# LemonATsu/UNet-PhaseGen

Hardware: AMD Instinct MI355X
Metric: spectrogram-frames/sec (train fwd+bwd) (higher is better)
Workload: dtype f32; 1 GPU; train.py full step (fwd + cos/sin/mag loss + bwd + Adam), UNetModel(1024, 2048), per-GPU batch 64 x 1024 bins x 256 frames (BASELINE configs[2]); global_batch=64, frames=256, channels=1024, parallelism=dp1, grad_allreduce_payload=fp32, adam=fused into the wgrad epilogues

## Files before the change

### unet-phasegen_amd/csrc/conv_raw_wgrad.hip

```cpp
#include "conv_common.h"

namespace {

template <int KW, int S> struct GRaw {
    static constexpr int WL = 15 * S + KW;
    static constexpr int WLP = g_wlp(KW, S);
    static constexpr int NQT = RBN / KW;
    static constexpr int TNV = NQT * KW;
    static constexpr int SUB = NQT * WLP;
    static constexpr int SUBS = (SUB + 63) / 64 * 64;
    static constexpr int NE = (SUB + NT - 1) / NT;
    static constexpr int STG = RTILE_A + 2 * SUBS;
    static constexpr int SUBP = (SUB + 255) / 256 * 256;
    static_assert(WL <= WLP, "window does not fit its slot");
};

template <int KW, int S, int BF>
__device__ __forceinline__ void g_raw_bf(const IgemmParams& p) {
    using C = GRaw<KW, S>;
    __shared__ __attribute__((aligned(16))) float lds[2 * C::STG];
    const int tid = threadIdx.x, lane = tid & 63;
    const int wv = __builtin_amdgcn_readfirstlane(tid >> 6), wm = wv >> 1, wn = wv & 1;
    const int kt = dma_kt(lane, wv);
    const rsrc_t rp = make_rsrc(p.pt, p.pt_bytes), rx = make_rsrc(p.x, p.x_bytes);
// ... 50 lines not shown
            }
        }
        int bbase[4];
#pragma unroll
        for (int jb = 0; jb < 4; ++jb) {
            const int c = wn * 128 + jb * 32 + (lane & 31), qc = c / KW;
            bbase[jb] = qc * C::WLP + (c - qc * KW) + S * 8 * (lane >> 5);
        }
        AccR acc;
#pragma unroll
        for (int i = 0; i < 2; ++i)
#pragma unroll
            for (int j = 0; j < 4; ++j)
#pragma unroll
                for (int r = 0; r < 16; ++r) acc.c[i][j][r] = 0.f;

        int gb, gi;
        { const int k0 = sb * BK; gb = k0 / p.LP; gi = k0 - gb * p.LP; }
        int kc_cur = 16;

#define GRAW_ISSUE(STAGE_PTR, K0)                                                                         \
    {   float* const As = (STAGE_PTR) + wv * 64; float* const Bw = (STAGE_PTR) + RTILE_A + wv * 64;       \
        const int k0 = (K0);                                                                              \
        const int kc = p.LP - gi;                            \
        if (FASTP && kc >= 16 && gb < p.B) {                                                              \
            const int sa = gb * pbs4 + gi * 4;                                                            \
            _Pragma("unroll") for (int e = 0; e < 2; ++e) dma16s(rp, As + wv * 192 + e * 1024, pv[FASTP ? e : 0], sa); \
        } else {                                                                                          \
          int bb, ii; divmod24(k0 + kt, p.LP, p.inv_LP, bb, ii);                                          \
          const int po = bb < p.B ? bb * pbs4 + ii * 4 : OOB;                                             \
          _Pragma("unroll") for (int e = 0; e < 8; ++e) dma4(rp, As + e * 256, aoff[e] + po); }           \
        const int w0 = S * gi - p.p;                             \
        if (FASTW && kc >= 16 && gb < p.B && w0 >= 0 && w0 + C::WLP <= p.Lx) {    \
            const int sw_ = gb * xbs4 + w0 * 4;                                                           \
            _Pragma("unroll") for (int e = 0; e < NE16; ++e)                                              \
                if (4 * (e * NT + wv * 64) < C::SUB) dma16s(rx, (STAGE_PTR) + RTILE_A + 4 * (e * NT + wv * 64), woff[FASTW ? e : 0], sw_); \
        } else {                                                                                          \
        const int sb0 = gb < p.B ? gb * xbs4 : -NEVER, sb1 = (kc < 16 && gb + 1 < p.B) ? (gb + 1) * xbs4 : -NEVER; \
        _Pragma("unroll") for (int e = 0; e < C::NE; ++e) {                                               \
            if ((e + 1) * NT <= C::SUB || e * NT + wv * 64 < C::SUB) {                                    \
                const int ps = S * gi + GRAW_VV(e);                                                       \
                dma4(rx, Bw + e * NT, ((unsigned)ps < (unsigned)p.Lx && sb0 >= 0) ? sb0 + GRAW_CHOFF(e) + ps * 4 : FAR); \
            }                                                                                             \
        }                                                                                                 \
        if (kc < 16) {                                  \
            _Pragma("unroll") for (int e = 0; e < C::NE; ++e) {                                           \
                if ((e + 1) * NT <= C::SUB || e * NT + wv * 64 < C::SUB) {                                                          \
                    const int ps = GRAW_VV(e);                                                            \
                    dma4(rx, Bw + C::SUBS + e * NT, ((unsigned)ps < (unsigned)p.Lx && sb1 >= 0) ? sb1 + GRAW_CHOFF(e) + ps * 4 : FAR); \
                }                                                                                         \
            }                                                                                             \
        }                                                                                                 \
        }                                                                                                 \
        kc_next = kc < 16 ? kc : 16;                                                                      \
        gi += BK; if (gi >= p.LP) { gi -= p.LP; ++gb; }                                                   \
    }

        PG_STAMP_DECL
        int kc_next;
        GRAW_ISSUE(lds, sb * BK)
        kc_cur = kc_next;
        __syncthreads();
        for (int sl = sb; sl < se; ++sl) {
            const int cur = (sl - sb) & 1;
            PG_STAMP(0)
#if defined(PG_G_ABL) && PG_G_ABL == 1
            kc_next = 16;
#else
            GRAW_ISSUE(lds + (cur ^ 1) * C::STG, (sl + 1) * BK)
#endif
            __builtin_amdgcn_sched_barrier(0);
            PG_STAMP(1)
            {
                const float* As = lds + cur * C::STG;
                const float* Bw = As + RTILE_A;
                const int r = lane & 31, h = lane >> 5, sw = (r >> 2) & 3;
                const float* ap = As + (wm * 64 + r) * BK;
                f32x4 a[2][2];
                float b[4][8];
                if (kc_cur >= 16) {
#pragma unroll
                    for (int i = 0; i < 2; ++i) a[i][0] = *reinterpret_cast<const f32x4*>(ap + i * 32 * BK + (((2 * h) ^ sw) << 2));
#pragma unroll
                    for (int ip = 0; ip < 4; ++ip) {
                        if (ip == 2) {
#pragma unroll
                            for (int i = 0; i < 2; ++i) a[i][1] = *reinterpret_cast<const f32x4*>(ap + i * 32 * BK + (((2 * h + 1) ^ sw) << 2));
                        }
#pragma unroll
                        for (int jb = 0; jb < 4; ++jb) { b[jb][2 * ip] = Bw[bbase[jb] + S * 2 * ip]; b[jb][2 * ip + 1] = Bw[bbase[jb] + S * (2 * ip + 1)]; }
                    }
                } else {
#pragma unroll
                    for (int c = 0; c < 2; ++c)
#pragma unroll
                        for (int i = 0; i < 2; ++i) a[i][c] = *reinterpret_cast<const f32x4*>(ap + i * 32 * BK + (((2 * h + c) ^ sw) << 2));
                    typedef const volatile __attribute__((address_space(3))) float* lds_vptr;
                    const lds_vptr Bv = (lds_vptr)Bw;
                    const int shift = C::SUBS - S * kc_cur;
#pragma unroll
                    for (int i = 0; i < 8; ++i) {
                        const int d = (8 * h + i >= kc_cur) ? shift : 0;
#pragma unroll
                        for (int jb = 0; jb < 4; ++jb) b[jb][i] = Bv[bbase[jb] + S * i + d];
                    }
                }
                if (slopeA != 1.0f) {
#pragma unroll
                    for (int i = 0; i < 2; ++i)
#pragma unroll
                        for (int c = 0; c < 2; ++c)
#pragma unroll
                            for (int v = 0; v < 4; ++v) a[i][c][v] = act_apply(a[i][c][v], slopeA);
                }
                if (slopeB != 1.0f) {
#pragma unroll
                    for (int jb = 0; jb < 4; ++jb)
#pragma unroll
                        for (int i = 0; i < 8; ++i) b[jb][i] = act_apply(b[jb][i], slopeB);
                }
                if (BF) mfma_low_2x4<BF>(a, b, acc);
                else {
#pragma unroll
                    for (int kk = 0; kk < 8; ++kk) {
#pragma unroll
                        for (int i = 0; i < 2; ++i)
#pragma unroll
                            for (int j = 0; j < 4; ++j)
                                acc.c[i][j] = __builtin_amdgcn_mfma_f32_32x32x2f32(a[i][kk >> 2][kk & 3], b[j][kk], acc.c[i][j], 0, 0, 0);
                    }
                }
            }
            __builtin_amdgcn_sched_barrier(0);
            PG_STAMP(2)
            kc_cur = kc_next;
#if defined(PG_G_ABL) && PG_G_ABL == 2
            asm volatile("s_waitcnt lgkmcnt(0)\n\ts_barrier" ::: "memory");
#else
            __syncthreads();
#endif
            PG_STAMP(3)
        }
        PG_STAMP_FLUSH
#undef GRAW_ISSUE
#undef GRAW_CHOFF
#undef GRAW_VV
        if (sb == 0 && se == p.nslab) epilogue_g<S, 2, 4>(p, acc, m0, n0, lane, wm, wn, n0 + C::TNV);
        else store_partial(p.ws, g, slot, acc, tid);
        pos += se - sb;
        slot = 1;
    }
}

template <int KW, int S, int BF>
__device__ __forceinline__ void g_ps_bf(const IgemmParams& p) {
    using C = GRaw<KW, S>;
    constexpr int STG = RTILE_A + (C::SUB + 255) / 256 * 256;
    constexpr int NE16 = (C::SUB / 4 + NT - 1) / NT;
    static_assert(C::WLP % 4 == 0 && C::WLP <= 64, "16-byte window pieces; channel 0 inside the first 64 floats");
    __shared__ __attribute__((aligned(16))) float lds[2 * STG];
    const int tid = threadIdx.x, lane = tid & 63;
    const int wv = __builtin_amdgcn_readfirstlane(tid >> 6), wm = wv >> 1, wn = wv & 1;
    const rsrc_t rp = make_rsrc(p.pt, p.pt_bytes), rx = make_rsrc(p.x, p.x_bytes);
    const float slopeA = act_slope(p.act_p), slopeB = act_slope(p.act_x);
    const int pbs4 = (int)p.pt_bs * 4, xbs4 = (int)p.x_bs * 4;
    const int cps = (p.LP + 15) >> 4;
    const int g = logical_wg(blockIdx.x, gridDim.x, p.whole);
    const Split sp = make_split(p.tilesM * p.tilesN, p.nslab, gridDim.x, p.whole);
    int pos = split_lo(sp, g);
    const int pos_end = split_lo(sp, g + 1);
    int slot = 0;
    while (pos < pos_end) {
        const int tile = pos / p.nslab, sb = pos - tile * p.nslab;
        const int se = min(p.nslab, sb + (pos_end - pos));
        const int m0 = (tile / p.tilesN) * RBM, n0 = (tile % p.tilesN) * C::TNV;
        const int qbase = (tile % p.tilesN) * C::NQT;

        int pv[2], woff[NE16];
#pragma unroll
        for (int e = 0; e < 2; ++e) {
            const int m = m0 + dma16_row(lane, wv, e);
            pv[e] = m < p.M ? (m * p.LP + dma16_kc(lane)) * 4 : FAR;
        }
#pragma unroll
        for (int e = 0; e < NE16; ++e) {
            const int f = 4 * (tid + NT * e), ql = f / C::WLP, v0 = f - ql * C::WLP;
            const int off = ((qbase + ql) * p.Lx + v0 - p.p) * 4;
            woff[e] = (f < C::SUB && qbase + ql < p.Q && off >= 0) ? off : FAR;
        }
        const bool fix0 = qbase == 0 && wv == 0;
        int f0_off, f0_v;
        { const int ql = lane / C::WLP, v = lane - ql * C::WLP; f0_off = ql < p.Q ? ql * p.Lx * 4 : FAR; f0_v = v - p.p; }
        int bbase[4], pj[4];
#pragma unroll
        for (int jb = 0; jb < 4; ++jb) {
            const int c = wn * 128 + jb * 32 + (lane & 31), qc = c / KW;
            bbase[jb] = qc * C::WLP + (c - qc * KW) + S * 8 * (lane >> 5);
            pj[jb] = (c - qc * KW) + S * 8 * (lane >> 5) - p.p;
        }
        AccR acc;
#pragma unroll
        for (int i = 0; i < 2; ++i)
#pragma unroll
            for (int j = 0; j < 4; ++j)
#pragma unroll
                for (int r = 0; r < 16; ++r) acc.c[i][j][r] = 0.f;

        int gb = sb / cps, gc = sb - gb * cps;
#define GPS_ISSUE(STAGE_PTR)                                                                              \
    {   float* const As = (STAGE_PTR) + wv * 64;                                                          \
        if (gb < p.B) {                                                                                   \
            const int gi = gc << 4;                                                                       \
            const int sa = gb * pbs4 + gi * 4;                                                            \
            _Pragma("unroll") for (int e = 0; e < 2; ++e) dma16s(rp, As + wv * 192 + e * 1024, pv[e], sa); \
            const int sw_ = gb * xbs4 + S * gi * 4;                                                       \
            _Pragma("unroll") for (int e = 0; e < NE16; ++e)                                              \
                if (4 * (e * NT + wv * 64) < C::SUB) dma16s(rx, (STAGE_PTR) + RTILE_A + 4 * (e * NT + wv * 64), woff[e], sw_); \
            if (fix0) {                                                                                   \
                const int ps = S * gi + f0_v;                                                             \
                dma4(rx, (STAGE_PTR) + RTILE_A, (unsigned)ps < (unsigned)p.Lx ? gb * xbs4 + f0_off + ps * 4 : FAR); \
            }                                                                                             \
        }                                                                                                 \
        if (++gc == cps) { gc = 0; ++gb; }                                                                \
    }
        int mb = gb, mc = gc;
        GPS_ISSUE(lds)
        __syncthreads();
        for (int sl = sb; sl < se; ++sl) {
            const int cur = (sl - sb) & 1;
            GPS_ISSUE(lds + (cur ^ 1) * STG)
            __builtin_amdgcn_sched_barrier(0);
            {
                const float* As = lds + cur * STG;
                const float* Bw = As + RTILE_A;
                const int r = lane & 31, h = lane >> 5, sw = (r >> 2) & 3;
                const float* ap = As + (wm * 64 + r) * BK;
                const int gi = mc << 4, kc = p.LP - gi;
                const int w0 = S * gi;
                f32x4 a[2][2];
                float b[4][8];
#pragma unroll
                for (int i = 0; i < 2; ++i) a[i][0] = *reinterpret_cast<const f32x4*>(ap + i * 32 * BK + (((2 * h) ^ sw) << 2));
#pragma unroll
                for (int ip = 0; ip < 4; ++ip) {
                    if (ip == 2) {
#pragma unroll
                        for (int i = 0; i < 2; ++i) a[i][1] = *reinterpret_cast<const f32x4*>(ap + i * 32 * BK + (((2 * h + 1) ^ sw) << 2));
                    }
#pragma unroll
                    for (int jb = 0; jb < 4; ++jb) { b[jb][2 * ip] = Bw[bbase[jb] + S * 2 * ip]; b[jb][2 * ip + 1] = Bw[bbase[jb] + S * (2 * ip + 1)]; }
                }
                if (kc < 16) {
#pragma unroll
                    for (int i = 0; i < 2; ++i)
#pragma unroll
                        for (int c = 0; c < 2; ++c)
#pragma unroll
                            for (int v = 0; v < 4; ++v) a[i][c][v] = (8 * h + 4 * c + v < kc) ? a[i][c][v] : 0.f;
                }
                if (w0 < p.p || w0 - p.p + C::WLP > p.Lx) {
#pragma unroll
                    for (int jb = 0; jb < 4; ++jb)
#pragma unroll
                        for (int i = 0; i < 8; ++i) b[jb][i] = (unsigned)(w0 + pj[jb] + S * i) < (unsigned)p.Lx ? b[jb][i] : 0.f;
                }
                if (slopeA != 1.0f) {
#pragma unroll
                    for (int i = 0; i < 2; ++i)
#pragma unroll
                        for (int c = 0; c < 2; ++c)
#pragma unroll
                            for (int v = 0; v < 4; ++v) a[i][c][v] = act_apply(a[i][c][v], slopeA);
                }
                if (slopeB != 1.0f) {
#pragma unroll
                    for (int jb = 0; jb < 4; ++jb)
#pragma unroll
                        for (int i = 0; i < 8; ++i) b[jb][i] = act_apply(b[jb][i], slopeB);
                }
                if (BF) mfma_low_2x4<BF>(a, b, acc);
                else {
#pragma unroll
                    for (int kk = 0; kk < 8; ++kk)
#pragma unroll
                        for (int i = 0; i < 2; ++i)
#pragma unroll
                            for (int j = 0; j < 4; ++j)
                                acc.c[i][j] = __builtin_amdgcn_mfma_f32_32x32x2f32(a[i][kk >> 2][kk & 3], b[j][kk], acc.c[i][j], 0, 0, 0);
                }
            }
            __builtin_amdgcn_sched_barrier(0);
            if (++mc == cps) { mc = 0; ++mb; }
            __syncthreads();
        }
#undef GPS_ISSUE
        (void)mb;
        if (sb == 0 && se == p.nslab) epilogue_g<S, 2, 4>(p, acc, m0, n0, lane, wm, wn, n0 + C::TNV);
        else store_partial(p.ws, g, slot, acc, tid);
        pos += se - sb;
        slot = 1;
    }
}

template <int KW, int S>
__device__ __forceinline__ void g_raw_f32(const IgemmParams& p) {
    using C = GRaw<KW, S>;
    constexpr int NP = 2 * C::SUBP / 4;
    constexpr int NE2 = (NP + NT - 1) / NT;
    constexpr int STG = RTILE_A + 2 * C::SUBP;
    static_assert(C::WLP % 4 == 0 && 2 * STG * 4 <= 64 * 1024, "16-byte window pieces; LDS budget");
    __shared__ __attribute__((aligned(16))) float lds[2 * STG];
    const int tid = threadIdx.x, lane = tid & 63;
    const int wv = __builtin_amdgcn_readfirstlane(tid >> 6), wm = wv >> 1, wn = wv & 1;
    const rsrc_t rp = make_rsrc(p.pk, p.pk_bytes), rx = make_rsrc(p.qk, p.qk_bytes);
    const int qbs4 = p.qk_bs * 4, klast4 = (p.nslab - 1) * BK * 4;
    const int g = logical_wg(blockIdx.x, gridDim.x, p.whole);
    const Split sp = make_split(p.tilesM * p.tilesN, p.nslab, gridDim.x, p.whole);
    int pos = split_lo(sp, g);
    const int pos_end = split_lo(sp, g + 1);
    int slot = 0;
    while (pos < pos_end) {
        const int tile = pos / p.nslab, sb = pos - tile * p.nslab;
        const int se = min(p.nslab, sb + (pos_end - pos));
        const int m0 = (tile / p.tilesN) * RBM, n0 = (tile % p.tilesN) * C::TNV;
        const int qbase = (tile % p.tilesN) * C::NQT;
        int pv[2], woff[NE2];
#pragma unroll
        for (int e = 0; e < 2; ++e) {
            const int m = m0 + dma16_row(lane, wv, e);
            pv[e] = m < p.M ? (m * p.Kp + dma16_kc(lane)) * 4 : FAR;
        }
#pragma unroll
        for (int e = 0; e < NE2; ++e) {
            const int pc = tid + NT * e, sub = pc >= C::SUBP / 4 ? 1 : 0, f = 4 * pc - sub * C::SUBP, ql = f / C::WLP, v0 = f - ql * C::WLP;
            woff[e] = (f < C::SUB && qbase + ql < p.Q) ? ((qbase + ql) * p.Lq + v0) * 4 : FAR;
        }
        int bbase[4];
#pragma unroll
        for (int jb = 0; jb < 4; ++jb) {
            const int c = wn * 128 + jb * 32 + (lane & 31), qc = c / KW;
            bbase[jb] = qc * C::WLP + (c - qc * KW) + S * 8 * (lane >> 5);
        }
        AccR acc;
#pragma unroll
        for (int i = 0; i < 2; ++i)
#pragma unroll
            for (int j = 0; j < 4; ++j)
#pragma unroll
                for (int r = 0; r < 16; ++r) acc.c[i][j][r] = 0.f;

        int gb, gi;
        { const int k0 = sb * BK; gb = k0 / p.LP; gi = k0 - gb * p.LP; }
        int kc_cur, kc_next;
#define GRF_ISSUE(STAGE_PTR, K0)                                                                          \
    {   const int sa = min((K0) * 4, klast4);                                                             \
        _Pragma("unroll") for (int e = 0; e < 2; ++e) dma16s(rp, (STAGE_PTR) + wv * 256 + e * 1024, pv[e], sa); \
        const int kc = p.LP - gi;                                                                         \
        const int sw0 = min(gb, p.B - 1) * qbs4 + S * gi * 4;                                             \
        const int sw1 = (kc < 16 && gb + 1 < p.B) ? (gb + 1) * qbs4 : sw0;                                \
        _Pragma("unroll") for (int e = 0; e < NE2; ++e) {                                                 \
            const int pc0 = e * NT + wv * 64;                                 \
            if ((e + 1) * NT <= NP || pc0 < NP)                                                           \
                dma16s(rx, (STAGE_PTR) + RTILE_A + 4 * pc0, woff[e], pc0 >= C::SUBP / 4 ? sw1 : sw0);     \
        }                                                                                                 \
        kc_next = kc < 16 ? kc : 16;                                                                      \
        gi += BK; if (gi >= p.LP) { gi -= p.LP; ++gb; }                                                   \
    }
        PG_STAMP_DECL
        GRF_ISSUE(lds, sb * BK)
        kc_cur = kc_next;
        __syncthreads();
        for (int sl = sb; sl < se; ++sl) {
            const int cur = (sl - sb) & 1;
            PG_STAMP(0)
#if defined(PG_G_ABL) && PG_G_ABL == 1
            kc_next = 16;
#else
            GRF_ISSUE(lds + (cur ^ 1) * STG, (sl + 1) * BK)
#endif
            __builtin_amdgcn_sched_barrier(0);
            PG_STAMP(1)
            {
                const float* As = lds + cur * STG;
                const float* Bw = As + RTILE_A;
                const int r = lane & 31, h = lane >> 5, sw = (r >> 2) & 3;
                const float* ap = As + (wm * 64 + r) * BK;
                f32x4 a[2][2];
                float b[4][8];
                if (kc_cur >= 16) {
#pragma unroll
                    for (int i = 0; i < 2; ++i) a[i][0] = *reinterpret_cast<const f32x4*>(ap + i * 32 * BK + (((2 * h) ^ sw) << 2));
#pragma unroll
                    for (int ip = 0; ip < 4; ++ip) {
                        if (ip == 2) {
#pragma unroll
                            for (int i = 0; i < 2; ++i) a[i][1] = *reinterpret_cast<const f32x4*>(ap + i * 32 * BK + (((2 * h + 1) ^ sw) << 2));
                        }
#pragma unroll
                        for (int jb = 0; jb < 4; ++jb) { b[jb][2 * ip] = Bw[bbase[jb] + S * 2 * ip]; b[jb][2 * ip + 1] = Bw[bbase[jb] + S * (2 * ip + 1)]; }
                    }
                } else {
#pragma unroll
                    for (int c = 0; c < 2; ++c)
#pragma unroll
                        for (int i = 0; i < 2; ++i) a[i][c] = *reinterpret_cast<const f32x4*>(ap + i * 32 * BK + (((2 * h + c) ^ sw) << 2));
                    typedef const volatile __attribute__((address_space(3))) float* lds_vptr;
                    const lds_vptr Bv = (lds_vptr)Bw;
                    const int shift = C::SUBP - S * kc_cur;
#pragma unroll
                    for (int i = 0; i < 8; ++i) {
                        const int d = (8 * h + i >= kc_cur) ? shift : 0;
#pragma unroll
                        for (int jb = 0; jb < 4; ++jb) b[jb][i] = Bv[bbase[jb] + S * i + d];
                    }
                }
#pragma unroll
                for (int kk = 0; kk < 8; ++kk)
#pragma unroll
                    for (int i = 0; i < 2; ++i)
#pragma unroll
                        for (int j = 0; j < 4; ++j)
                            acc.c[i][j] = __builtin_amdgcn_mfma_f32_32x32x2f32(a[i][kk >> 2][kk & 3], b[j][kk], acc.c[i][j], 0, 0, 0);
            }
            __builtin_amdgcn_sched_barrier(0);
            PG_STAMP(2)
            kc_cur = kc_next;
            __syncthreads();
            PG_STAMP(3)
        }
        PG_STAMP_FLUSH
#undef GRF_ISSUE
        if (sb == 0 && se == p.nslab) epilogue_g<S, 2, 4>(p, acc, m0, n0, lane, wm, wn, n0 + C::TNV);
        else store_partial(p.ws, g, slot, acc, tid);
        pos += se - sb;
        slot = 1;
    }
}

template <int KW, int S>
__device__ __forceinline__ void g_ps_f32(const IgemmParams& p) {
    using C = GRaw<KW, S>;
    constexpr int STG = RTILE_A + (C::SUB + 255) / 256 * 256;
    constexpr int NE16 = (C::SUB / 4 + NT - 1) / NT;
    static_assert(C::WLP % 4 == 0, "16-byte window pieces");
    __shared__ __attribute__((aligned(16))) float lds[2 * STG];
    const int tid = threadIdx.x, lane = tid & 63;
    const int wv = __builtin_amdgcn_readfirstlane(tid >> 6), wm = wv >> 1, wn = wv & 1;
    const rsrc_t rp = make_rsrc(p.pk, p.pk_bytes), rx = make_rsrc(p.qk, p.qk_bytes);
    const int pbs4 = p.M * p.Kp * 4, qbs4 = p.qk_bs * 4;
    const int cps = p.Kp >> 4;
    const int g = logical_wg(blockIdx.x, gridDim.x, p.whole);
    const Split sp = make_split(p.tilesM * p.tilesN, p.nslab, gridDim.x, p.whole);
    int pos = split_lo(sp, g);
    const int pos_end = split_lo(sp, g + 1);
    int slot = 0;
    while (pos < pos_end) {
        const int tile = pos / p.nslab, sb = pos - tile * p.nslab;
        const int se = min(p.nslab, sb + (pos_end - pos));
        const int m0 = (tile / p.tilesN) * RBM, n0 = (tile % p.tilesN) * C::TNV;
        const int qbase = (tile % p.tilesN) * C::NQT;
        int pv[2], woff[NE16];
#pragma unroll
        for (int e = 0; e < 2; ++e) {
            const int m = m0 + dma16_row(lane, wv, e);
            pv[e] = m < p.M ? (m * p.Kp + dma16_kc(lane)) * 4 : FAR;
        }
#pragma unroll
        for (int e = 0; e < NE16; ++e) {
            const int f = 4 * (tid + NT * e), ql = f / C::WLP, v0 = f - ql * C::WLP;
            woff[e] = (f < C::SUB && qbase + ql < p.Q) ? ((qbase + ql) * p.Lq + v0) * 4 : FAR;
        }
        int bbase[4];
#pragma unroll
        for (int jb = 0; jb < 4; ++jb) {
            const int c = wn * 128 + jb * 32 + (lane & 31), qc = c / KW;
            bbase[jb] = qc * C::WLP + (c - qc * KW) + S * 8 * (lane >> 5);
        }
        AccR acc;
#pragma unroll
        for (int i = 0; i < 2; ++i)
#pragma unroll
            for (int j = 0; j < 4; ++j)
#pragma unroll
                for (int r = 0; r < 16; ++r) acc.c[i][j][r] = 0.f;

        int gb = sb / cps, gc = sb - gb * cps;
#define GPF_ISSUE(STAGE_PTR)                                                                              \
    {   const int gbc = min(gb, p.B - 1), gi = gc << 4;                                                   \
        _Pragma("unroll") for (int e = 0; e < 2; ++e) dma16s(rp, (STAGE_PTR) + wv * 256 + e * 1024, pv[e], gbc * pbs4 + gi * 4); \
        const int sw_ = gbc * qbs4 + S * gi * 4;                                                          \
        _Pragma("unroll") for (int e = 0; e < NE16; ++e)                                                  \
            if (4 * (e * NT + wv * 64) < C::SUB) dma16s(rx, (STAGE_PTR) + RTILE_A + 4 * (e * NT + wv * 64), woff[e], sw_); \
        if (++gc == cps) { gc = 0; ++gb; }                                                                \
    }
        GPF_ISSUE(lds)
        __syncthreads();
        for (int sl = sb; sl < se; ++sl) {
            const int cur = (sl - sb) & 1;
            GPF_ISSUE(lds + (cur ^ 1) * STG)
            __builtin_amdgcn_sched_barrier(0);
            {
                const float* As = lds + cur * STG;
                const float* Bw = As + RTILE_A;
                const int r = lane & 31, h = lane >> 5, sw = (r >> 2) & 3;
                const float* ap = As + (wm * 64 + r) * BK;
                f32x4 a[2][2];
                float b[4][8];
#pragma unroll
                for (int i = 0; i < 2; ++i) a[i][0] = *reinterpret_cast<const f32x4*>(ap + i * 32 * BK + (((2 * h) ^ sw) << 2));
#pragma unroll
                for (int ip = 0; ip < 4; ++ip) {
                    if (ip == 2) {
#pragma unroll
                        for (int i = 0; i < 2; ++i) a[i][1] = *reinterpret_cast<const f32x4*>(ap + i * 32 * BK + (((2 * h + 1) ^ sw) << 2));
                    }
#pragma unroll
                    for (int jb = 0; jb < 4; ++jb) { b[jb][2 * ip] = Bw[bbase[jb] + S * 2 * ip]; b[jb][2 * ip + 1] = Bw[bbase[jb] + S * (2 * ip + 1)]; }
                }
#pragma unroll
                for (int kk = 0; kk < 8; ++kk)
#pragma unroll
                    for (int i = 0; i < 2; ++i)
#pragma unroll
                        for (int j = 0; j < 4; ++j)
                            acc.c[i][j] = __builtin_amdgcn_mfma_f32_32x32x2f32(a[i][kk >> 2][kk & 3], b[j][kk], acc.c[i][j], 0, 0, 0);
            }
            __builtin_amdgcn_sched_barrier(0);
            __syncthreads();
        }
#undef GPF_ISSUE
        if (sb == 0 && se == p.nslab) epilogue_g<S, 2, 4>(p, acc, m0, n0, lane, wm, wn, n0 + C::TNV);
        else store_partial(p.ws, g, slot, acc, tid);
        pos += se - sb;
        slot = 1;
    }
}

template <int KW, int S, int BF>
__global__ __launch_bounds__(NT, 2) void conv_g_raw_kernel(const IgemmParams p) {
    if constexpr (BF == 0) g_raw_f32<KW, S>(p);
    else g_raw_bf<KW, S, BF>(p);
}
template <int KW, int S, int BF>
__global__ __launch_bounds__(NT, 2) void conv_g_ps_kernel(const IgemmParams p) {
    if constexpr (BF == 0) g_ps_f32<KW, S>(p);
    else g_ps_bf<KW, S, BF>(p);
}

__global__ __launch_bounds__(256) void pack_rows_kernel(const float* __restrict__ src, long bs, int C, int L, int F, int W, unsigned n,
                                                       float slope, float* __restrict__ dst) {
    for (unsigned i = blockIdx.x * 256u + threadIdx.x; i < n; i += gridDim.x * 256u) {
        const unsigned r = i / (unsigned)W, b = r / (unsigned)C, c = r - b * (unsigned)C;
        const int t = (int)(i - r * (unsigned)W) - F;
        float v = 0.f;
        if ((unsigned)t < (unsigned)L) {
            v = src[(long)b * bs + (long)c * L + t];
            if (slope != 1.0f) v = act_apply(v, slope);
        }
        dst[i] = v;
    }
}
__global__ __launch_bounds__(256) void pack_flat_kernel(const float* __restrict__ src, long bs, int B, int LP, int Kp, unsigned n,
                                                       float slope, float* __restrict__ dst) {
    for (unsigned i = blockIdx.x * 256u + threadIdx.x; i < n; i += gridDim.x * 256u) {
        const unsigned m = i / (unsigned)Kp, k = i - m * (unsigned)Kp, b = k / (unsigned)LP, t = k - b * (unsigned)LP;
        float v = 0.f;
        if ((int)b < B) {
            v = src[(long)b * bs + (long)m * LP + t];
            if (slope != 1.0f) v = act_apply(v, slope);
        }
        dst[i] = v;
    }
}
unsigned pack_grid(unsigned n) { return (n + 255u) / 256u < 2048u ? (n + 255u) / 256u : 2048u; }

hipError_t pack_g(const IgemmParams& p, hipStream_t st) {
    float* const qk = const_cast<float*>(p.qk);
    float* const pk = const_cast<float*>(p.pk);
    const unsigned nq = (unsigned)(p.qk_bytes / 4), np = (unsigned)(p.pk_bytes / 4);
    hipLaunchKernelGGL(pack_rows_kernel, dim3(pack_grid(nq)), dim3(256), 0, st, p.x, p.x_bs, p.Q, p.Lx, p.p, p.Lq, nq, act_slope(p.act_x), qk);
    if (p.g_ps) hipLaunchKernelGGL(pack_rows_kernel, dim3(pack_grid(np)), dim3(256), 0, st, p.pt, p.pt_bs, p.M, p.LP, 0, p.Kp, np, act_slope(p.act_p), pk);
    else hipLaunchKernelGGL(pack_flat_kernel, dim3(pack_grid(np)), dim3(256), 0, st, p.pt, p.pt_bs, p.B, p.LP, p.Kp, np, act_slope(p.act_p), pk);
    return hipGetLastError();
}

template <int KW, int S>
hipError_t launch_g_raw(const IgemmParams& p, int grid, hipStream_t st, int prec) {
    if (prec == 0) {
        if (hipError_t e = pack_g(p, st)) return e;
    }
    if (p.g_ps) {
        if (prec == 1) hipLaunchKernelGGL((conv_g_ps_kernel<KW, S, 1>), dim3(grid), dim3(NT), 0, st, p);
        else if (prec == 2) hipLaunchKernelGGL((conv_g_ps_kernel<KW, S, 2>), dim3(grid), dim3(NT), 0, st, p);
        else hipLaunchKernelGGL((conv_g_ps_kernel<KW, S, 0>), dim3(grid), dim3(NT), 0, st, p);
        return hipGetLastError();
    }
    if (prec == 1) hipLaunchKernelGGL((conv_g_raw_kernel<KW, S, 1>), dim3(grid), dim3(NT), 0, st, p);
    else if (prec == 2) hipLaunchKernelGGL((conv_g_raw_kernel<KW, S, 2>), dim3(grid), dim3(NT), 0, st, p);
    else hipLaunchKernelGGL((conv_g_raw_kernel<KW, S, 0>), dim3(grid), dim3(NT), 0, st, p);
    return hipGetLastError();
}

}

hipError_t pgconv::launch_raw_g(const IgemmParams& p, int grid, hipStream_t st, int prec) {
    if (p.k == 32) return launch_g_raw<32, 2>(p, grid, st, prec);
    if (p.k == 8 && p.s == 1) return launch_g_raw<8, 1>(p, grid, st, prec);
    if (p.k == 8) return launch_g_raw<8, 2>(p, grid, st, prec);
    if (p.k == 5) return launch_g_raw<5, 2>(p, grid, st, prec);
    return launch_g_raw<4, 2>(p, grid, st, prec);
}
```

Measured before the change: 99040 frames/s.

## Rewrite fp32 weight-gradient kernels as 2-wave, 3-stage ring with interleaved LDS reads

The fp32 raw and per-sample weight-gradient conv kernels are replaced by one templated kernel. It uses 128 threads (2 waves) with 4x4 MFMA tiles per wave and a 3-slot LDS ring in dynamic shared memory. Each MFMA chunk is interleaved by hand with the next fragment's LDS reads and the global gather issues, using explicit vmcnt and lgkmcnt waits. The pack kernels are also rewritten to work per row with 16-byte stores. The aim is to hide LDS and global latency behind MFMA work. In exchange the code relies on hand-written asm scheduling, higher register use per wave and lower occupancy, which adds complexity and may cause correctness or spill risk.

```diff
diff --git a/unet-phasegen_amd/csrc/conv_raw_wgrad.hip b/unet-phasegen_amd/csrc/conv_raw_wgrad.hip
--- a/unet-phasegen_amd/csrc/conv_raw_wgrad.hip
+++ b/unet-phasegen_amd/csrc/conv_raw_wgrad.hip
@@ -376,150 +376,130 @@
     }
 }
 
-template <int KW, int S>
-__device__ __forceinline__ void g_raw_f32(const IgemmParams& p) {
+constexpr int NT1 = 128;
+constexpr int G1_RING = 3;
+constexpr int G1_SLOTS = 8;
+
+template <int N> __device__ __forceinline__ void g1_wait_vmcnt() {
+    static_assert(N >= 0 && N < 64, "vmcnt is a 6-bit count");
+    __builtin_amdgcn_s_waitcnt((N & 15) | ((N >> 4) << 14) | (7 << 4) | (15 << 8));
+}
+__device__ __forceinline__ void g1_lgkm0() { __builtin_amdgcn_s_waitcnt(0xc07f); }
+__device__ __forceinline__ unsigned g1_lds_addr(const float* p) {
+    return (unsigned)(size_t)(const __attribute__((address_space(3))) float*)p;
+}
+__device__ __forceinline__ float g1_acc(float v) {
+    float x;
+    asm volatile("v_accvgpr_read_b32 %0, %1" : "=v"(x) : "a"(v));
+    return x;
+}
+
+template <int KW, int S, bool FLAT> struct G1 {
     using C = GRaw<KW, S>;
-    constexpr int NP = 2 * C::SUBP / 4;
-    constexpr int NE2 = (NP + NT - 1) / NT;
-    constexpr int STG = RTILE_A + 2 * C::SUBP;
-    static_assert(C::WLP % 4 == 0 && 2 * STG * 4 <= 64 * 1024, "16-byte window pieces; LDS budget");
-    __shared__ __attribute__((aligned(16))) float lds[2 * STG];
-    const int tid = threadIdx.x, lane = tid & 63;
-    const int wv = __builtin_amdgcn_readfirstlane(tid >> 6), wm = wv >> 1, wn = wv & 1;
-    const rsrc_t rp = make_rsrc(p.pk, p.pk_bytes), rx = make_rsrc(p.qk, p.qk_bytes);
-    const int qbs4 = p.qk_bs * 4, klast4 = (p.nslab - 1) * BK * 4;
-    const int g = logical_wg(blockIdx.x, gridDim.x, p.whole);
-    const Split sp = make_split(p.tilesM * p.tilesN, p.nslab, gridDim.x, p.whole);
-    int pos = split_lo(sp, g);
-    const int pos_end = split_lo(sp, g + 1);
-    int slot = 0;
-    while (pos < pos_end) {
-        const int tile = pos / p.nslab, sb = pos - tile * p.nslab;
-        const int se = min(p.nslab, sb + (pos_end - pos));
-        const int m0 = (tile / p.tilesN) * RBM, n0 = (tile % p.tilesN) * C::TNV;
-        const int qbase = (tile % p.tilesN) * C::NQT;
-        int pv[2], woff[NE2];
-#pragma unroll
-        for (int e = 0; e < 2; ++e) {
-            const int m = m0 + dma16_row(lane, wv, e);
-            pv[e] = m < p.M ? (m * p.Kp + dma16_kc(lane)) * 4 : FAR;
-        }
-#pragma unroll
-        for (int e = 0; e < NE2; ++e) {
-            const int pc = tid + NT * e, sub = pc >= C::SUBP / 4 ? 1 : 0, f = 4 * pc - sub * C::SUBP, ql = f / C::WLP, v0 = f - ql * C::WLP;
-            woff[e] = (f < C::SUB && qbase + ql < p.Q) ? ((qbase + ql) * p.Lq + v0) * 4 : FAR;
-        }
-        int bbase[4];
-#pragma unroll
-        for (int jb = 0; jb < 4; ++jb) {
-            const int c = wn * 128 + jb * 32 + (lane & 31), qc = c / KW;
-            bbase[jb] = qc * C::WLP + (c - qc * KW) + S * 8 * (lane >> 5);
-        }
-        AccR acc;
-#pragma unroll
-        for (int i = 0; i < 2; ++i)
-#pragma unroll
-            for (int j = 0; j < 4; ++j)
-#pragma unroll
-                for (int r = 0; r < 16; ++r) acc.c[i][j][r] = 0.f;
-
-        int gb, gi;
-        { const int k0 = sb * BK; gb = k0 / p.LP; gi = k0 - gb * p.LP; }
-        int kc_cur, kc_next;
-#define GRF_ISSUE(STAGE_PTR, K0)                                                                          \
-    {   const int sa = min((K0) * 4, klast4);                                                             \
-        _Pragma("unroll") for (int e = 0; e < 2; ++e) dma16s(rp, (STAGE_PTR) + wv * 256 + e * 1024, pv[e], sa); \
-        const int kc = p.LP - gi;                                                                         \
-        const int sw0 = min(gb, p.B - 1) * qbs4 + S * gi * 4;                                             \
-        const int sw1 = (kc < 16 && gb + 1 < p.B) ? (gb + 1) * qbs4 : sw0;                                \
-        _Pragma("unroll") for (int e = 0; e < NE2; ++e) {                                                 \
-            const int pc0 = e * NT + wv * 64;                                 \
-            if ((e + 1) * NT <= NP || pc0 < NP)                                                           \
-                dma16s(rx, (STAGE_PTR) + RTILE_A + 4 * pc0, woff[e], pc0 >= C::SUBP / 4 ? sw1 : sw0);     \
-        }                                                                                                 \
-        kc_next = kc < 16 ? kc : 16;                                                                      \
-        gi += BK; if (gi >= p.LP) { gi -= p.LP; ++gb; }                                                   \
-    }
-        PG_STAMP_DECL
-        GRF_ISSUE(lds, sb * BK)
-        kc_cur = kc_next;
-        __syncthreads();
-        for (int sl = sb; sl < se; ++sl) {
-            const int cur = (sl - sb) & 1;
-            PG_STAMP(0)
-#if defined(PG_G_ABL) && PG_G_ABL == 1
-            kc_next = 16;
+    static constexpr int WIN = FLAT ? 2 * C::SUBP : C::SUBP;
+    static constexpr int STG = RTILE_A + WIN;
+    static constexpr int NI = WIN / 256;
+    static constexpr int NW = (NI + 1) / 2;
+    static constexpr int ND = 4 + NW;
+    static constexpr int ND0 = ND < G1_SLOTS ? ND : G1_SLOTS;
+    static constexpr int LDS_BYTES = G1_RING * STG * 4;
+    static constexpr bool UNI = 32 % KW == 0;
+    static constexpr int JBS = UNI ? (32 / KW) * C::WLP : 0;
+    static_assert(C::WLP % 4 == 0 && C::SUBP % 256 == 0, "16-byte window pieces, whole wave instructions per sub-window");
+    static_assert(ND <= 2 * G1_SLOTS && 2 * ND < 64, "gather slots per slab / vmcnt range");
+    static_assert(2 * LDS_BYTES <= 160 * 1024, "two workgroups per CU");
+};
+
+struct G1Frag { f32x4 a[4]; float b[4][4]; };
+struct G1Addr { unsigned a0, ab; int t; unsigned shift4; };
+template <int KW, int S, bool FLAT, int NC>
+__device__ __forceinline__ G1Addr g1_addr(const float* stage, int r, int h, int bb0, int kc) {
+    G1Addr A;
+    A.a0 = g1_lds_addr(stage) + (r * 16 + (((2 * h + NC) ^ ((r >> 2) & 3)) << 2)) * 4;
+    A.ab = g1_lds_addr(stage + RTILE_A) + bb0 * 4;
+    A.t = kc - 8 * h - 4 * NC;
+    A.shift4 = (unsigned)((GRaw<KW, S>::SUBP - S * kc) * 4);
+    return A;
+}
+template <int KW, int S, bool FLAT, int NC, int CI>
+__device__ __forceinline__ void g1_load_b(const G1Addr& A, unsigned (&ae)[4], const int (&dj)[4], G1Frag& f) {
+    using G = G1<KW, S, FLAT>;
+    constexpr int i = CI >> 2, jb = CI & 3;
+    if (jb == 0) ae[i] = FLAT ? A.ab + (i >= A.t ? A.shift4 : 0u) : A.ab;
+    if constexpr (G::UNI) asm volatile("ds_read_b32 %0, %1 offset:%2" : "=v"(f.b[jb][i]) : "v"(ae[i]), "n"((G::JBS * jb + S * (4 * NC + i)) * 4));
+    else asm volatile("ds_read_b32 %0, %1 offset:%2" : "=v"(f.b[jb][i]) : "v"(ae[i] + (unsigned)dj[jb]), "n"(S * (4 * NC + i) * 4));
+}
+template <int I> __device__ __forceinline__ void g1_load_a(const G1Addr& A, G1Frag& f) {
+    asm volatile("ds_read_b128 %0, %1 offset:%2" : "=v"(f.a[I]) : "v"(A.a0), "n"(I * 2048));
+}
+
+template <int KW, int S, bool FLAT, int CC, int E0, typename Issue>
+__device__ __forceinline__ void g1_half(const G1Frag& cur, G1Frag& nxt, const float* nstage, int r, int h, int bb0, const int (&dj)[4],
+                                        int kc, AccT<4, 4>& acc, const Issue& issue) {
+    constexpr int NC = 1 - CC;
+    const G1Addr A = g1_addr<KW, S, FLAT, NC>(nstage, r, h, bb0, kc);
+    unsigned ae[4];
+#define G1_CHUNK(C, WORK)                                                                                                        \
+    __builtin_amdgcn_sched_barrier(0);                                                                                           \
+    acc.c[((C) >> 2) & 3][(C) & 3] = __builtin_amdgcn_mfma_f32_32x32x2f32(cur.a[((C) >> 2) & 3][(C) >> 4], cur.b[(C) & 3][(C) >> 4], \
+                                                                          acc.c[((C) >> 2) & 3][(C) & 3], 0, 0, 0);              \
+    WORK;
+#define G1_ROW(C0, W0, W1, W2, W3) G1_CHUNK(C0, W0) G1_CHUNK(C0 + 1, W1) G1_CHUNK(C0 + 2, W2) G1_CHUNK(C0 + 3, W3)
+#define G1_LB(CI) (g1_load_b<KW, S, FLAT, NC, CI>(A, ae, dj, nxt))
+#if defined(PG_G_ABL) && PG_G_ABL == 4
+    (void)A; (void)ae;
+    G1_ROW(0, (void)0, (void)0, (void)0, (void)0)
+    G1_ROW(4, (void)0, (void)0, (void)0, (void)0)
+    G1_ROW(8, (void)0, (void)0, (void)0, (void)0)
+    G1_ROW(12, (void)0, (void)0, (void)0, (void)0)
+    G1_ROW(16, (void)0, (void)0, (void)0, (void)0)
 #else
-            GRF_ISSUE(lds + (cur ^ 1) * STG, (sl + 1) * BK)
+    G1_ROW(0, G1_LB(0), G1_LB(1), G1_LB(2), G1_LB(3))
+    G1_ROW(4, G1_LB(4), G1_LB(5), G1_LB(6), G1_LB(7))
+    G1_ROW(8, G1_LB(8), G1_LB(9), G1_LB(10), G1_LB(11))
+    G1_ROW(12, G1_LB(12), G1_LB(13), G1_LB(14), G1_LB(15))
+    G1_ROW(16, (g1_load_a<0>(A, nxt)), (g1_load_a<1>(A, nxt)), (g1_load_a<2>(A, nxt)), (g1_load_a<3>(A, nxt)))
 #endif
-            __builtin_amdgcn_sched_barrier(0);
-            PG_STAMP(1)
-            {
-                const float* As = lds + cur * STG;
-                const float* Bw = As + RTILE_A;
-                const int r = lane & 31, h = lane >> 5, sw = (r >> 2) & 3;
-                const float* ap = As + (wm * 64 + r) * BK;
-                f32x4 a[2][2];
-                float b[4][8];
-                if (kc_cur >= 16) {
-#pragma unroll
-                    for (int i = 0; i < 2; ++i) a[i][0] = *reinterpret_cast<const f32x4*>(ap + i * 32 * BK + (((2 * h) ^ sw) << 2));
-#pragma unroll
-                    for (int ip = 0; ip < 4; ++ip) {
-                        if (ip == 2) {
-#pragma unroll
-                            for (int i = 0; i < 2; ++i) a[i][1] = *reinterpret_cast<const f32x4*>(ap + i * 32 * BK + (((2 * h + 1) ^ sw) << 2));
-                        }
-#pragma unroll
-                        for (int jb = 0; jb < 4; ++jb) { b[jb][2 * ip] = Bw[bbase[jb] + S * 2 * ip]; b[jb][2 * ip + 1] = Bw[bbase[jb] + S * (2 * ip + 1)]; }
-                    }
-                } else {
-#pragma unroll
-                    for (int c = 0; c < 2; ++c)
-#pragma unroll
-                        for (int i = 0; i < 2; ++i) a[i][c] = *reinterpret_cast<const f32x4*>(ap + i * 32 * BK + (((2 * h + c) ^ sw) << 2));
-                    typedef const volatile __attribute__((address_space(3))) float* lds_vptr;
-                    const lds_vptr Bv = (lds_vptr)Bw;
-                    const int shift = C::SUBP - S * kc_cur;
-#pragma unroll
-                    for (int i = 0; i < 8; ++i) {
-                        const int d = (8 * h + i >= kc_cur) ? shift : 0;
-#pragma unroll
-                        for (int jb = 0; jb < 4; ++jb) b[jb][i] = Bv[bbase[jb] + S * i + d];
-                    }
-                }
-#pragma unroll
-                for (int kk = 0; kk < 8; ++kk)
-#pragma unroll
-                    for (int i = 0; i < 2; ++i)
-#pragma unroll
-                        for (int j = 0; j < 4; ++j)
-                            acc.c[i][j] = __builtin_amdgcn_mfma_f32_32x32x2f32(a[i][kk >> 2][kk & 3], b[j][kk], acc.c[i][j], 0, 0, 0);
-            }
-            __builtin_amdgcn_sched_barrier(0);
-            PG_STAMP(2)
-            kc_cur = kc_next;
-            __syncthreads();
-            PG_STAMP(3)
-        }
-        PG_STAMP_FLUSH
-#undef GRF_ISSUE
-        if (sb == 0 && se == p.nslab) epilogue_g<S, 2, 4>(p, acc, m0, n0, lane, wm, wn, n0 + C::TNV);
-        else store_partial(p.ws, g, slot, acc, tid);
-        pos += se - sb;
-        slot = 1;
-    }
-}
-
-template <int KW, int S>
-__device__ __forceinline__ void g_ps_f32(const IgemmParams& p) {
+    G1_ROW(20, issue(E0 + 0), (void)0, (void)0, (void)0)
+    G1_ROW(24, (void)0, issue(E0 + 1), (void)0, (void)0)
+    G1_ROW(28, (void)0, (void)0, issue(E0 + 2), (void)0)
+    G1_ROW(32, (void)0, (void)0, (void)0, issue(E0 + 3))
+    G1_ROW(36, (void)0, (void)0, (void)0, (void)0)
+    G1_ROW(40, issue(E0 + 4), (void)0, (void)0, (void)0)
+    G1_ROW(44, (void)0, issue(E0 + 5), (void)0, (void)0)
+    G1_ROW(48, (void)0, (void)0, issue(E0 + 6), (void)0)
+    G1_ROW(52, (void)0, (void)0, (void)0, issue(E0 + 7))
+    G1_ROW(56, (void)0, (void)0, (void)0, (void)0)
+#if defined(PG_G_ABL) && PG_G_ABL == 4
+    G1_ROW(60, (void)0, (void)0, (void)0, (void)0)
+    nxt = cur;
+#else
+    G1_ROW(60, g1_lgkm0(), (void)0, (void)0, (void)0)
+#endif
+    __builtin_amdgcn_sched_barrier(0);
+#undef G1_LB
+#undef G1_ROW
+#undef G1_CHUNK
+}
+
+__device__ __forceinline__ void store_partial_g1(float* ws, int g, int slot, const AccT<4, 4>& acc, int w, int lane) {
+    float* dst = ws + ((long)(g * 2 + slot) * ACC_REGS) * NT + lane;
+#pragma unroll
+    for (int i = 0; i < 4; ++i)
+#pragma unroll
+        for (int j = 0; j < 4; ++j)
+#pragma unroll
+            for (int r = 0; r < 16; ++r) dst[(((i & 1) * 4 + j) * 16 + r) * NT + ((i >> 1) * 2 + w) * 64] = g1_acc(acc.c[i][j][r]);
+}
+
+template <int KW, int S, bool FLAT>
+__device__ __forceinline__ void g1_f32(const IgemmParams& p) {
     using C = GRaw<KW, S>;
-    constexpr int STG = RTILE_A + (C::SUB + 255) / 256 * 256;
-    constexpr int NE16 = (C::SUB / 4 + NT - 1) / NT;
-    static_assert(C::WLP % 4 == 0, "16-byte window pieces");
-    __shared__ __attribute__((aligned(16))) float lds[2 * STG];
-    const int tid = threadIdx.x, lane = tid & 63;
-    const int wv = __builtin_amdgcn_readfirstlane(tid >> 6), wm = wv >> 1, wn = wv & 1;
+    using G = G1<KW, S, FLAT>;
+    constexpr int STG = G::STG, ND = G::ND, ND0 = G::ND0;
+    extern __shared__ __attribute__((aligned(16))) float lds[];
+    const int lane = threadIdx.x & 63, r = lane & 31, h = lane >> 5;
+    const int w = __builtin_amdgcn_readfirstlane(threadIdx.x >> 6);
     const rsrc_t rp = make_rsrc(p.pk, p.pk_bytes), rx = make_rsrc(p.qk, p.qk_bytes);
     const int pbs4 = p.M * p.Kp * 4, qbs4 = p.qk_bs * 4;
     const int cps = p.Kp >> 4;
@@ -533,128 +513,205 @@
         const int se = min(p.nslab, sb + (pos_end - pos));
         const int m0 = (tile / p.tilesN) * RBM, n0 = (tile % p.tilesN) * C::TNV;
         const int qbase = (tile % p.tilesN) * C::NQT;
-        int pv[2], woff[NE16];
-#pragma unroll
-        for (int e = 0; e < 2; ++e) {
-            const int m = m0 + dma16_row(lane, wv, e);
+        int pv[4], woff[G::NW];
+#pragma unroll
+        for (int e = 0; e < 4; ++e) {
+            const int m = m0 + (2 * e + w) * 16 + (lane >> 2);
             pv[e] = m < p.M ? (m * p.Kp + dma16_kc(lane)) * 4 : FAR;
         }
 #pragma unroll
-        for (int e = 0; e < NE16; ++e) {
-            const int f = 4 * (tid + NT * e), ql = f / C::WLP, v0 = f - ql * C::WLP;
+        for (int e = 0; e < G::NW; ++e) {
+            const int x = 2 * e + w < G::NI ? 2 * e + w : w;
+            const int pc = x * 64 + lane, sub = (FLAT && pc >= C::SUBP / 4) ? 1 : 0, f = 4 * pc - sub * C::SUBP, ql = f / C::WLP, v0 = f - ql * C::WLP;
             woff[e] = (f < C::SUB && qbase + ql < p.Q) ? ((qbase + ql) * p.Lq + v0) * 4 : FAR;
         }
-        int bbase[4];
-#pragma unroll
-        for (int jb = 0; jb < 4; ++jb) {
-            const int c = wn * 128 + jb * 32 + (lane & 31), qc = c / KW;
-            bbase[jb] = qc * C::WLP + (c - qc * KW) + S * 8 * (lane >> 5);
-        }
-        AccR acc;
-#pragma unroll
-        for (int i = 0; i < 2; ++i)
+        int bb0, dj[4];
+        {
+            int bbase[4];
+#pragma unroll
+            for (int jb = 0; jb < 4; ++jb) {
+                const int c = w * 128 + jb * 32 + r, qc = c / KW;
+                bbase[jb] = qc * C::WLP + (c - qc * KW) + S * 8 * h;
+            }
+            bb0 = bbase[0];
+#pragma unroll
+            for (int jb = 0; jb < 4; ++jb) dj[jb] = (bbase[jb] - bb0) * 4;
+        }
+        AccT<4, 4> acc;
+#pragma unroll
+        for (int i = 0; i < 4; ++i)
 #pragma unroll
             for (int j = 0; j < 4; ++j)
 #pragma unroll
-                for (int r = 0; r < 16; ++r) acc.c[i][j][r] = 0.f;
-
-        int gb = sb / cps, gc = sb - gb * cps;
-#define GPF_ISSUE(STAGE_PTR)                                                                              \
-    {   const int gbc = min(gb, p.B - 1), gi = gc << 4;                                                   \
-        _Pragma("unroll") for (int e = 0; e < 2; ++e) dma16s(rp, (STAGE_PTR) + wv * 256 + e * 1024, pv[e], gbc * pbs4 + gi * 4); \
-        const int sw_ = gbc * qbs4 + S * gi * 4;                                                          \
-        _Pragma("unroll") for (int e = 0; e < NE16; ++e)                                                  \
-            if (4 * (e * NT + wv * 64) < C::SUB) dma16s(rx, (STAGE_PTR) + RTILE_A + 4 * (e * NT + wv * 64), woff[e], sw_); \
-        if (++gc == cps) { gc = 0; ++gb; }                                                                \
-    }
-        GPF_ISSUE(lds)
+                for (int q = 0; q < 16; ++q) acc.c[i][j][q] = 0.f;
+
+        int gb, gi;
+        if (FLAT) { const int k0 = sb * BK; gb = k0 / p.LP; gi = k0 - gb * p.LP; }
+        else { gb = sb / cps; gi = sb - gb * cps; }
+        int ri = gi;
+        int sa, sw0, sw1, gslab = sb;
+        auto next_slab = [&]() {
+            if (FLAT) {
+                const int kc = p.LP - gi;
+                sa = gslab * (BK * 4);
+                sw0 = gb * qbs4 + S * gi * 4;
+                sw1 = (kc < 16 && gb + 1 < p.B) ? (gb + 1) * qbs4 : sw0;
+                gi += BK; if (gi >= p.LP) { gi -= p.LP; ++gb; }
+            } else {
+                sa = gb * pbs4 + gi * (BK * 4);
+                sw0 = sw1 = gb * qbs4 + S * gi * (BK * 4);
+                if (++gi == cps) { gi = 0; ++gb; }
+            }
+            ++gslab;
+        };
+        auto issue_piece = [&](float* stage, bool live, bool inloop, int e) {
+#if defined(PG_G_ABL) && (PG_G_ABL == 1 || PG_G_ABL == 4)
+            if (inloop) return;
+#endif
+            if (e < 4) dma16s(rp, stage + (2 * e + w) * 256, live ? pv[e < 4 ? e : 0] : FAR, sa);
+            else if (e < ND) {
+                const int ew = e - 4, x = 2 * ew + w < G::NI ? 2 * ew + w : w;
+                dma16s(rx, stage + RTILE_A + x * 256, live ? woff[ew < G::NW ? ew : 0] : FAR, (FLAT && x * 64 >= C::SUBP / 4) ? sw1 : sw0);
+            }
+        };
+        g1_wait_vmcnt<0>();
+#pragma unroll
+        for (int hf = 0; hf < 2; ++hf) {
+            next_slab();
+#pragma unroll
+            for (int e = 0; e < ND; ++e) issue_piece(lds + hf * STG, sb + hf < se, false, e);
+        }
+        __builtin_amdgcn_sched_barrier(0);
+        g1_wait_vmcnt<ND>();
+        __builtin_amdgcn_s_barrier();
+        asm volatile("" ::: "memory");
+        int kc_cur = FLAT ? p.LP - ri : 16;
+        G1Frag f0, f1;
+        {
+            const G1Addr A = g1_addr<KW, S, FLAT, 0>(lds, r, h, bb0, kc_cur);
+            unsigned ae[4];
+#define G1_LB(CI) g1_load_b<KW, S, FLAT, 0, CI>(A, ae, dj, f0);
+            G1_LB(0) G1_LB(1) G1_LB(2) G1_LB(3) G1_LB(4) G1_LB(5) G1_LB(6) G1_LB(7)
+            G1_LB(8) G1_LB(9) G1_LB(10) G1_LB(11) G1_LB(12) G1_LB(13) G1_LB(14) G1_LB(15)
+#undef G1_LB
+            g1_load_a<0>(A, f0); g1_load_a<1>(A, f0); g1_load_a<2>(A, f0); g1_load_a<3>(A, f0);
+            g1_lgkm0();
+            __builtin_amdgcn_sched_barrier(0);
+        }
+        int st = 0;
+        for (int sl = sb; sl < se; ++sl) {
+            const int st1 = st == 2 ? 0 : st + 1, st2 = st >= 1 ? st - 1 : 2;
+            float* const ring2 = lds + st2 * STG;
+            const bool live2 = sl + 2 < se;
+            next_slab();
+            auto issue0 = [&](int e) { if (e < ND0) issue_piece(ring2, live2, true, e); };
+            auto issue1 = [&](int e) { if (e < ND) issue_piece(ring2, live2, true, e); };
+            g1_half<KW, S, FLAT, 0, 0>(f0, f1, lds + st * STG, r, h, bb0, dj, kc_cur, acc, issue0);
+            if (FLAT) { ri += BK; if (ri >= p.LP) ri -= p.LP; kc_cur = p.LP - ri; }
+#if defined(PG_G_ABL)
+            g1_wait_vmcnt<0>();
+#else
+            g1_wait_vmcnt<ND0>();
+#endif
+            __builtin_amdgcn_s_barrier();
+            asm volatile("" ::: "memory");
+            g1_half<KW, S, FLAT, 1, ND0>(f1, f0, lds + st1 * STG, r, h, bb0, dj, kc_cur, acc, issue1);
+            st = st1;
+        }
+        g1_wait_vmcnt<0>();
         __syncthreads();
-        for (int sl = sb; sl < se; ++sl) {
-            const int cur = (sl - sb) & 1;
-            GPF_ISSUE(lds + (cur ^ 1) * STG)
-            __builtin_amdgcn_sched_barrier(0);
-            {
-                const float* As = lds + cur * STG;
-                const float* Bw = As + RTILE_A;
-                const int r = lane & 31, h = lane >> 5, sw = (r >> 2) & 3;
-                const float* ap = As + (wm * 64 + r) * BK;
-                f32x4 a[2][2];
-                float b[4][8];
-#pragma unroll
-                for (int i = 0; i < 2; ++i) a[i][0] = *reinterpret_cast<const f32x4*>(ap + i * 32 * BK + (((2 * h) ^ sw) << 2));
-#pragma unroll
-                for (int ip = 0; ip < 4; ++ip) {
-                    if (ip == 2) {
-#pragma unroll
-                        for (int i = 0; i < 2; ++i) a[i][1] = *reinterpret_cast<const f32x4*>(ap + i * 32 * BK + (((2 * h + 1) ^ sw) << 2));
-                    }
-#pragma unroll
-                    for (int jb = 0; jb < 4; ++jb) { b[jb][2 * ip] = Bw[bbase[jb] + S * 2 * ip]; b[jb][2 * ip + 1] = Bw[bbase[jb] + S * (2 * ip + 1)]; }
-                }
-#pragma unroll
-                for (int kk = 0; kk < 8; ++kk)
-#pragma unroll
-                    for (int i = 0; i < 2; ++i)
-#pragma unroll
-                        for (int j = 0; j < 4; ++j)
-                            acc.c[i][j] = __builtin_amdgcn_mfma_f32_32x32x2f32(a[i][kk >> 2][kk & 3], b[j][kk], acc.c[i][j], 0, 0, 0);
-            }
-            __builtin_amdgcn_sched_barrier(0);
-            __syncthreads();
-        }
-#undef GPF_ISSUE
-        if (sb == 0 && se == p.nslab) epilogue_g<S, 2, 4>(p, acc, m0, n0, lane, wm, wn, n0 + C::TNV);
-        else store_partial(p.ws, g, slot, acc, tid);
+        asm volatile("s_nop 15\n\ts_nop 15\n\ts_nop 15\n\ts_nop 15\n\ts_nop 15");
+        if (sb == 0 && se == p.nslab) {
+#define G1_EPI(I, J)                                                                                              \
+    {   AccT<1, 1> blk;                                                                                          \
+        _Pragma("unroll") for (int q = 0; q < 16; ++q) blk.c[0][0][q] = g1_acc(acc.c[I][J][q]);                  \
+        __builtin_amdgcn_sched_barrier(0);                                                                       \
+        epilogue_g<S, 1, 1>(p, blk, m0 + (I) * 32, n0 + (w * 4 + (J)) * 32, lane, 0, 0, n0 + C::TNV);            \
+        __builtin_amdgcn_sched_barrier(0);                                                                       \
+    }
+            G1_EPI(0, 0) G1_EPI(0, 1) G1_EPI(0, 2) G1_EPI(0, 3) G1_EPI(1, 0) G1_EPI(1, 1) G1_EPI(1, 2) G1_EPI(1, 3)
+            G1_EPI(2, 0) G1_EPI(2, 1) G1_EPI(2, 2) G1_EPI(2, 3) G1_EPI(3, 0) G1_EPI(3, 1) G1_EPI(3, 2) G1_EPI(3, 3)
+#undef G1_EPI
+        } else store_partial_g1(p.ws, g, slot, acc, w, lane);
         pos += se - sb;
         slot = 1;
     }
 }
 
 template <int KW, int S, int BF>
-__global__ __launch_bounds__(NT, 2) void conv_g_raw_kernel(const IgemmParams p) {
-    if constexpr (BF == 0) g_raw_f32<KW, S>(p);
+__global__ __launch_bounds__(BF == 0 ? NT1 : NT, BF == 0 ? 1 : 2) void conv_g_raw_kernel(const IgemmParams p) {
+    if constexpr (BF == 0) g1_f32<KW, S, true>(p);
     else g_raw_bf<KW, S, BF>(p);
 }
 template <int KW, int S, int BF>
-__global__ __launch_bounds__(NT, 2) void conv_g_ps_kernel(const IgemmParams p) {
-    if constexpr (BF == 0) g_ps_f32<KW, S>(p);
+__global__ __launch_bounds__(BF == 0 ? NT1 : NT, BF == 0 ? 1 : 2) void conv_g_ps_kernel(const IgemmParams p) {
+    if constexpr (BF == 0) g1_f32<KW, S, false>(p);
     else g_ps_bf<KW, S, BF>(p);
 }
 
-__global__ __launch_bounds__(256) void pack_rows_kernel(const float* __restrict__ src, long bs, int C, int L, int F, int W, unsigned n,
+__global__ __launch_bounds__(256) void pack_rows_kernel(const float* __restrict__ src, long bs, int C, int L, int F, int W, unsigned rows,
                                                        float slope, float* __restrict__ dst) {
-    for (unsigned i = blockIdx.x * 256u + threadIdx.x; i < n; i += gridDim.x * 256u) {
-        const unsigned r = i / (unsigned)W, b = r / (unsigned)C, c = r - b * (unsigned)C;
-        const int t = (int)(i - r * (unsigned)W) - F;
-        float v = 0.f;
-        if ((unsigned)t < (unsigned)L) {
-            v = src[(long)b * bs + (long)c * L + t];
-            if (slope != 1.0f) v = act_apply(v, slope);
-        }
-        dst[i] = v;
-    }
-}
-__global__ __launch_bounds__(256) void pack_flat_kernel(const float* __restrict__ src, long bs, int B, int LP, int Kp, unsigned n,
+    const int lane = threadIdx.x & 63;
+    for (unsigned r = __builtin_amdgcn_readfirstlane(blockIdx.x * 4u + (threadIdx.x >> 6)); r < rows; r += gridDim.x * 4u) {
+        const unsigned b = r / (unsigned)C, c = r - b * (unsigned)C;
+        const float* s = src + (long)b * bs + (long)c * L;
+        float* d = dst + (size_t)r * W;
+        for (int j = 4 * lane; j < W; j += 256) {
+            f32x4 v;
+#pragma unroll
+            for (int e = 0; e < 4; ++e) {
+                const int t = j + e - F;
+                float x = 0.f;
+                if ((unsigned)t < (unsigned)L) {
+                    x = s[t];
+                    if (slope != 1.0f) x = act_apply(x, slope);
+                }
+                v[e] = x;
+            }
+            *reinterpret_cast<f32x4*>(d + j) = v;
+        }
+    }
+}
+__global__ __launch_bounds__(256) void pack_flat_kernel(const float* __restrict__ src, long bs, int B, int LP, int Kp, unsigned rows,
                                                        float slope, float* __restrict__ dst) {
-    for (unsigned i = blockIdx.x * 256u + threadIdx.x; i < n; i += gridDim.x * 256u) {
-        const unsigned m = i / (unsigned)Kp, k = i - m * (unsigned)Kp, b = k / (unsigned)LP, t = k - b * (unsigned)LP;
-        float v = 0.f;
-        if ((int)b < B) {
-            v = src[(long)b * bs + (long)m * LP + t];
-            if (slope != 1.0f) v = act_apply(v, slope);
-        }
-        dst[i] = v;
-    }
-}
-unsigned pack_grid(unsigned n) { return (n + 255u) / 256u < 2048u ? (n + 255u) / 256u : 2048u; }
+    for (unsigned m = blockIdx.x; m < rows; m += gridDim.x) {
+        const float* s = src + (long)m * LP;
+        float* d = dst + (size_t)m * Kp;
+        for (int k = 4 * threadIdx.x; k < Kp; k += 1024) {
+            int b = k / LP, t = k - b * LP;
+            f32x4 v;
+#pragma unroll
+            for (int e = 0; e < 4; ++e) {
+                float x = 0.f;
+                if (b < B) {
+                    x = s[(long)b * bs + t];
+                    if (slope != 1.0f) x = act_apply(x, slope);
+                }
+                v[e] = x;
+                if (++t == LP) { t = 0; ++b; }
+            }
+            *reinterpret_cast<f32x4*>(d + k) = v;
+        }
+    }
+}
+unsigned pack_grid(unsigned blocks) { return blocks < 8192u ? blocks : 8192u; }
 
 hipError_t pack_g(const IgemmParams& p, hipStream_t st) {
     float* const qk = const_cast<float*>(p.qk);
     float* const pk = const_cast<float*>(p.pk);
-    const unsigned nq = (unsigned)(p.qk_bytes / 4), np = (unsigned)(p.pk_bytes / 4);
-    hipLaunchKernelGGL(pack_rows_kernel, dim3(pack_grid(nq)), dim3(256), 0, st, p.x, p.x_bs, p.Q, p.Lx, p.p, p.Lq, nq, act_slope(p.act_x), qk);
-    if (p.g_ps) hipLaunchKernelGGL(pack_rows_kernel, dim3(pack_grid(np)), dim3(256), 0, st, p.pt, p.pt_bs, p.M, p.LP, 0, p.Kp, np, act_slope(p.act_p), pk);
-    else hipLaunchKernelGGL(pack_flat_kernel, dim3(pack_grid(np)), dim3(256), 0, st, p.pt, p.pt_bs, p.B, p.LP, p.Kp, np, act_slope(p.act_p), pk);
+    const unsigned rq = (unsigned)(p.qk_bytes / 4) / (unsigned)p.Lq, rp = (unsigned)(p.pk_bytes / 4) / (unsigned)p.Kp;
+    hipLaunchKernelGGL(pack_rows_kernel, dim3(pack_grid((rq + 3) / 4)), dim3(256), 0, st, p.x, p.x_bs, p.Q, p.Lx, p.p, p.Lq, rq, act_slope(p.act_x), qk);
+    if (p.g_ps) hipLaunchKernelGGL(pack_rows_kernel, dim3(pack_grid((rp + 3) / 4)), dim3(256), 0, st, p.pt, p.pt_bs, p.M, p.LP, 0, p.Kp, rp, act_slope(p.act_p), pk);
+    else hipLaunchKernelGGL(pack_flat_kernel, dim3(pack_grid(rp)), dim3(256), 0, st, p.pt, p.pt_bs, p.B, p.LP, p.Kp, rp, act_slope(p.act_p), pk);
+    return hipGetLastError();
+}
+
+template <int LDS_BYTES>
+hipError_t launch_g1(void (*kern)(const IgemmParams), const IgemmParams& p, int grid, hipStream_t st) {
+    if (LDS_BYTES > 48 * 1024) {
+        if (hipError_t e = hipFuncSetAttribute((const void*)kern, hipFuncAttributeMaxDynamicSharedMemorySize, LDS_BYTES)) return e;
+    }
+    hipLaunchKernelGGL(kern, dim3(grid), dim3(NT1), LDS_BYTES, st, p);
     return hipGetLastError();
 }
 
@@ -666,12 +723,12 @@
     if (p.g_ps) {
         if (prec == 1) hipLaunchKernelGGL((conv_g_ps_kernel<KW, S, 1>), dim3(grid), dim3(NT), 0, st, p);
         else if (prec == 2) hipLaunchKernelGGL((conv_g_ps_kernel<KW, S, 2>), dim3(grid), dim3(NT), 0, st, p);
-        else hipLaunchKernelGGL((conv_g_ps_kernel<KW, S, 0>), dim3(grid), dim3(NT), 0, st, p);
+        else return launch_g1<G1<KW, S, false>::LDS_BYTES>(conv_g_ps_kernel<KW, S, 0>, p, grid, st);
         return hipGetLastError();
     }
     if (prec == 1) hipLaunchKernelGGL((conv_g_raw_kernel<KW, S, 1>), dim3(grid), dim3(NT), 0, st, p);
     else if (prec == 2) hipLaunchKernelGGL((conv_g_raw_kernel<KW, S, 2>), dim3(grid), dim3(NT), 0, st, p);
-    else hipLaunchKernelGGL((conv_g_raw_kernel<KW, S, 0>), dim3(grid), dim3(NT), 0, st, p);
+    else return launch_g1<G1<KW, S, true>::LDS_BYTES>(conv_g_raw_kernel<KW, S, 0>, p, grid, st);
     return hipGetLastError();
 }
 
```

Measured after the change: 97810 frames/s. 1.2% lower.
